# cordum-io/cordum

Measured on AMD Instinct MI355X. Metric: jobs dispatched/sec (whole node), higher is better.
Workload: dtype int64-bitset/int32 (control-plane integer path); 1 GPU; model=cordum control-plane dispatch pipeline (echo workers), global_batch=16384, seq_len=256, parallelism=shard1, rules=1024, workers_per_rank=1000, denied_jobs=14465

## Files before the change

cordum_amd/ops/hip/cordum_kernels.hip:

```cpp
#include <hip/hip_runtime.h>
#include <cstdint>

#define WAVE 64
#define BLOCK 256


template <int W, int JPT>
__global__ __launch_bounds__(BLOCK) void policy_first_match_kernel(
    const long long* __restrict__ rule_any,
    const long long* __restrict__ rule_all,
    const signed char* __restrict__ rule_secrets,
    const long long* __restrict__ rule_mcp,
    const unsigned char* __restrict__ rule_mcp_any,
    const long long* __restrict__ job_any,
    const long long* __restrict__ job_all,
    const unsigned char* __restrict__ job_secrets,
    const long long* __restrict__ job_mcp,
    const unsigned char* __restrict__ job_mcp_used,
    int* __restrict__ out_first,
    int R, int J, int rules_per_chunk)
{
    const int rule_chunk_begin = blockIdx.y * rules_per_chunk;
    const int rule_chunk_end = min(R, rule_chunk_begin + rules_per_chunk);
    constexpr int ANY_W = 7 * W;
// ... 1873 lines not shown
    #pragma unroll
    for (int t = 0; t < TJ; ++t) {
        const int job = (blockIdx.x * TJ + t) * 16 + (lane & 15);
        #pragma unroll
        for (int d = 0; d < 9; ++d) {
            unsigned long long w = 0;
            if (job < J)
                w = (unsigned long long)(d < 7 ? any_bits[(size_t)job * 7 + d]
                                               : all_bits[(size_t)job * 2 + (d - 7)]);
            const unsigned int slice = (unsigned int)(w >> shift) & 0xFFFFu;
            #pragma unroll
            for (int q = 0; q < 4; ++q)
                afrag[t][d][q] = (int)((((slice >> (4 * q)) & 0xFu) * 0x00204081u) & 0x01010101u);
        }
    }
    mfma_first_match_tiles<TJ>(afrag, b_pack, cards, rule_secrets, job_secrets,
                               tile_dims, out_first, J, R, tiles_per_chunk);
}

template <int TJ>
__global__ __launch_bounds__(BLOCK) void policy_first_match_mfma_cols_kernel(
    const long long* __restrict__ cols,
    int L, unsigned long long col_map,
    const signed char* __restrict__ b_pack,
    const int* __restrict__ cards,
    const signed char* __restrict__ rule_secrets,
    const unsigned char* __restrict__ job_secrets,
    const int* __restrict__ tile_dims,
    int* __restrict__ out_first,
    int J, int R, int tiles_per_chunk)
{
    const int lane = threadIdx.x % WAVE;
    const int shift = (lane >> 4) * 16;
    v4i afrag[TJ][9];
    #pragma unroll
    for (int t = 0; t < TJ; ++t) {
        const int job = (blockIdx.x * TJ + t) * 16 + (lane & 15);
        #pragma unroll
        for (int d = 0; d < 9; ++d) {
            const int c = (int)((col_map >> (4 * d)) & 0xFull);
            unsigned long long w = 0;
            if (c < L && job < J)
                w = (unsigned long long)cols[(size_t)job * L + c];
            const unsigned int slice = (unsigned int)(w >> shift) & 0xFFFFu;
            #pragma unroll
            for (int q = 0; q < 4; ++q)
                afrag[t][d][q] = (int)((((slice >> (4 * q)) & 0xFu) * 0x00204081u) & 0x01010101u);
        }
    }
    mfma_first_match_tiles<TJ>(afrag, b_pack, cards, rule_secrets, job_secrets,
                               tile_dims, out_first, J, R, tiles_per_chunk);
}


__global__ __launch_bounds__(BLOCK) void policy_gate_kernel(
    const int* __restrict__ first,
    const signed char* __restrict__ decisions,
    signed char* __restrict__ out_decision,
    int* __restrict__ denied_slots,
    int* __restrict__ denied_count,
    int* __restrict__ allowed_slots,
    int* __restrict__ allowed_count,
    int J, int R)
{
    const int j = blockIdx.x * BLOCK + threadIdx.x;
    const int lane = threadIdx.x % WAVE;
    gate_job(j, J, lane, first, decisions, R, out_decision,
             allowed_slots, allowed_count, denied_slots, denied_count);
}

__global__ __launch_bounds__(BLOCK) void policy_gate_full_kernel(
    const int* __restrict__ first,
    const signed char* __restrict__ decisions,
    signed char* __restrict__ out_decision,
    int* __restrict__ denied_slots,
    int* __restrict__ denied_count,
    int* __restrict__ allowed_slots,
    int* __restrict__ allowed_count,
    unsigned char* __restrict__ states,
    long long* __restrict__ deadlines,
    int* __restrict__ dlq_ring,
    int* __restrict__ dlq_head,
    int ring_size,
    int J, int R)
{
    const int j = blockIdx.x * BLOCK + threadIdx.x;
    const int lane = threadIdx.x % WAVE;
    const bool allowed = gate_job(j, J, lane, first, decisions, R, out_decision,
                                  allowed_slots, allowed_count, denied_slots, denied_count);
    deny_to_dlq(j < J && !allowed, j, lane, states, deadlines, dlq_ring, dlq_head, ring_size);
}

__global__ __launch_bounds__(BLOCK) void begin_tick_kernel(
    unsigned char* __restrict__ states, int B,
    int* __restrict__ counts, int ncounts,
    int* __restrict__ first)
{
    begin_slot(blockIdx.x * BLOCK + threadIdx.x, states, B, counts, ncounts, first);
}

__global__ void accumulate_counts_kernel(
    const int* __restrict__ counts, long long* __restrict__ acc, int n)
{
    const int t = threadIdx.x;
    if (t < n) acc[t] += (long long)counts[t];
}
// ... 856 lines not shown
    const int n = (int)counts.size(0);
    const int NW = (int)out_keys.size(0);
    TORCH_CHECK(w_active.size(0) == NW && w_maxp.size(0) == NW &&
                w_cpu.size(0) == NW && w_gpu.size(0) == NW, "worker table size mismatch");
    TORCH_CHECK(!first.has_value() || first->size(0) == B, "first must be [B]");
    const int blocks = (std::max(std::max(B, n), std::max(NW, 1)) + BLOCK - 1) / BLOCK;
    hipLaunchKernelGGL(tick_prologue_kernel, dim3(blocks), dim3(BLOCK), 0, cur_stream(),
        states.data_ptr<uint8_t>(), B, counts.data_ptr<int>(), n,
        first.has_value() ? first->data_ptr<int>() : (int*)nullptr,
        w_active.data_ptr<int>(), w_maxp.data_ptr<int>(),
        w_cpu.data_ptr<float>(), w_gpu.data_ptr<float>(),
        (unsigned long long*)out_keys.data_ptr<int64_t>(), NW);
}

void policy_first_match_mfma_bits_into(
    torch::Tensor any_bits, torch::Tensor all_bits,
    torch::Tensor b_pack, torch::Tensor cards,
    torch::Tensor rule_secrets, torch::Tensor job_secrets,
    torch::Tensor tile_dims, int64_t n_rules, torch::Tensor out, int64_t job_tiles)
{
    CHECK_DEV(any_bits); CHECK_DEV(b_pack);
    CHECK_CONTIG(any_bits); CHECK_CONTIG(all_bits);
    TORCH_CHECK(job_tiles == 1 || job_tiles == 2, "job_tiles must be 1 or 2");
    TORCH_CHECK(any_bits.dim() == 3 && any_bits.size(1) == 7 && any_bits.size(2) == 1 &&
                all_bits.dim() == 3 && all_bits.size(1) == 2 && all_bits.size(2) == 1,
                "MFMA K1 needs the 1-word vocab: any [J,7,1], all [J,2,1]");
    const int J = (int)any_bits.size(0), R = (int)n_rules;
    TORCH_CHECK(all_bits.size(0) == J && job_secrets.size(0) >= J && out.size(0) >= J,
                "job tensors must cover J");
    const int TJ = (int)job_tiles;
    const int Jt = ((J + 15) / 16 + TJ - 1) / TJ;
    const int Rt = (R + 15) / 16;
    if (J == 0 || R == 0) return;
    TORCH_CHECK(b_pack.size(0) >= Rt && tile_dims.size(0) >= Rt &&
                rule_secrets.size(0) >= Rt * 16 && cards.size(0) >= Rt * 16,
                "rule pack smaller than n_rules");
    int nchunks = std::max(1, std::min((Rt + 3) / 4, std::max(1, 2048 / std::max(Jt, 1))));
    const int tiles_per_chunk = (Rt + nchunks - 1) / nchunks;
    auto launch = [&](auto kernel) {
        hipLaunchKernelGGL(kernel, dim3(Jt, nchunks), dim3(BLOCK), 0, cur_stream(),
            (const long long*)any_bits.data_ptr<int64_t>(),
            (const long long*)all_bits.data_ptr<int64_t>(),
            (const signed char*)b_pack.data_ptr<int8_t>(),
            cards.data_ptr<int>(),
            (const signed char*)rule_secrets.data_ptr<int8_t>(),
            job_secrets.data_ptr<uint8_t>(),
            tile_dims.data_ptr<int>(),
            out.data_ptr<int>(), J, R, tiles_per_chunk);
    };
    if (TJ == 2) launch(policy_first_match_mfma_bits_kernel<2>);
    else launch(policy_first_match_mfma_bits_kernel<1>);
}

void policy_first_match_mfma_cols_into(
    torch::Tensor cols, int64_t col_map,
    torch::Tensor b_pack, torch::Tensor cards,
    torch::Tensor rule_secrets, torch::Tensor job_secrets,
    torch::Tensor tile_dims, int64_t n_rules, torch::Tensor out, int64_t job_tiles)
{
    CHECK_DEV(cols); CHECK_DEV(b_pack);
    CHECK_CONTIG(cols);
    TORCH_CHECK(job_tiles == 1 || job_tiles == 2, "job_tiles must be 1 or 2");
    TORCH_CHECK(cols.dim() == 2 && cols.scalar_type() == torch::kInt64 && cols.size(1) <= 9,
                "compact K1 needs cols [J,L] int64 with L <= 9 (1-word vocab)");
    const int J = (int)cols.size(0), R = (int)n_rules, L = (int)cols.size(1);
    TORCH_CHECK(job_secrets.size(0) >= J && out.size(0) >= J, "job tensors must cover J");
    TORCH_CHECK(col_map >= 0 && (col_map >> 36) == 0, "col_map holds 9 nibbles");
    unsigned map_dims = 0;
    int next_col = 0;
    for (int d = 0; d < 9; ++d) {
        const int c = (int)((col_map >> (4 * d)) & 0xF);
        if (c == 0xF) continue;
        TORCH_CHECK(c == next_col, "col_map must number the live dims 0..L-1 in ascending d");
        ++next_col;
        map_dims |= 1u << d;
    }
    TORCH_CHECK(next_col == L, "col_map names ", next_col, " columns, cols has ", L);
    const int TJ = (int)job_tiles;
    const int Jt = ((J + 15) / 16 + TJ - 1) / TJ;
    const int Rt = (R + 15) / 16;
    if (J == 0 || R == 0) return;
    TORCH_CHECK(b_pack.size(0) >= Rt && tile_dims.size(0) >= Rt &&
                rule_secrets.size(0) >= Rt * 16 && cards.size(0) >= Rt * 16,
                "rule pack smaller than n_rules");
    hipStreamCaptureStatus capturing = hipStreamCaptureStatusNone;
    TORCH_CHECK(hipStreamIsCapturing(cur_stream(), &capturing) == hipSuccess,
                "hipStreamIsCapturing failed");
    if (capturing == hipStreamCaptureStatusNone) {
        const torch::Tensor td = tile_dims.narrow(0, 0, Rt).cpu();
        const int* p = td.data_ptr<int>();
        unsigned scanned = 0;
        for (int rt = 0; rt < Rt; ++rt) scanned |= (unsigned)p[rt];
        TORCH_CHECK((scanned & 0x1FFu & ~map_dims) == 0,
                    "col_map lacks a dimension the packed policy scans (stale map?): "
                    "tile_dims union ", scanned & 0x1FFu, ", map dims ", map_dims);
    }
    int nchunks = std::max(1, std::min((Rt + 3) / 4, std::max(1, 2048 / std::max(Jt, 1))));
    const int tiles_per_chunk = (Rt + nchunks - 1) / nchunks;
    auto launch = [&](auto kernel) {
        hipLaunchKernelGGL(kernel, dim3(Jt, nchunks), dim3(BLOCK), 0, cur_stream(),
            (const long long*)cols.data_ptr<int64_t>(), L, (unsigned long long)col_map,
            (const signed char*)b_pack.data_ptr<int8_t>(),
            cards.data_ptr<int>(),
            (const signed char*)rule_secrets.data_ptr<int8_t>(),
            job_secrets.data_ptr<uint8_t>(),
            tile_dims.data_ptr<int>(),
            out.data_ptr<int>(), J, R, tiles_per_chunk);
    };
    if (TJ == 2) launch(policy_first_match_mfma_cols_kernel<2>);
    else launch(policy_first_match_mfma_cols_kernel<1>);
}

void gate_route(torch::Tensor first, torch::Tensor decisions, torch::Tensor out_decision,
                torch::Tensor denied_slots, torch::Tensor denied_count,
                torch::Tensor allowed_slots, torch::Tensor allowed_count,
                torch::Tensor states, torch::Tensor deadlines,
                torch::Tensor dlq_ring, torch::Tensor dlq_head,
                torch::Tensor pick, torch::Tensor order, torch::Tensor valid_count,
                torch::Tensor j_poolmask, torch::Tensor j_labels,
                int64_t full_mask, int64_t K,
                torch::Tensor routable_slots, torch::Tensor routable_widx,
                torch::Tensor routable_count, torch::Tensor extra_zero)
{
    CHECK_DEV(first);
    const int J = (int)first.size(0);
    TORCH_CHECK(out_decision.size(0) >= J && denied_slots.size(0) >= J &&
                allowed_slots.size(0) >= J && states.size(0) >= J &&
                deadlines.size(0) >= J && pick.size(0) >= J &&
                j_poolmask.size(0) >= J && j_labels.size(0) >= J &&
                routable_slots.size(0) >= J && routable_widx.size(0) >= J,
                "per-job tensors must cover J");
    TORCH_CHECK(K <= order.size(0), "K exceeds the order table");
    const int n_extra = (int)extra_zero.size(0);
    const int blocks = (std::max(std::max(J, n_extra), 1) + BLOCK - 1) / BLOCK;
    hipLaunchKernelGGL(gate_route_kernel, dim3(blocks), dim3(BLOCK), 0, cur_stream(),
        first.data_ptr<int>(), (const signed char*)decisions.data_ptr<int8_t>(),
        (signed char*)out_decision.data_ptr<int8_t>(),
        denied_slots.data_ptr<int>(), denied_count.data_ptr<int>(),
        allowed_slots.data_ptr<int>(), allowed_count.data_ptr<int>(),
        states.data_ptr<uint8_t>(), (long long*)deadlines.data_ptr<int64_t>(),
        dlq_ring.data_ptr<int>(), dlq_head.data_ptr<int>(), (int)dlq_ring.size(0),
        pick.data_ptr<int>(), order.data_ptr<int>(), valid_count.data_ptr<int>(),
        (const long long*)j_poolmask.data_ptr<int64_t>(),
        (const long long*)j_labels.data_ptr<int64_t>(),
        (long long)full_mask, (int)K,
        routable_slots.data_ptr<int>(), routable_widx.data_ptr<int>(),
        routable_count.data_ptr<int>(),
        extra_zero.data_ptr<int>(), n_extra,
        J, (int)decisions.size(0));
}

void tick_finish(torch::Tensor ctx_arena, torch::Tensor routable_slots,
                 torch::Tensor routable_widx, torch::Tensor routable_count,
                 torch::Tensor res_arena, torch::Tensor res_sum, int64_t stride,
                 torch::Tensor states, torch::Tensor attempts, torch::Tensor deadlines,
                 std::vector<int64_t> chain,
                 torch::Tensor w_active_local, int64_t nwl, int64_t my_rank,
                 torch::Tensor counts, torch::Tensor acc, int64_t capacity)
{
    CHECK_DEV(ctx_arena);
    TORCH_CHECK(capacity <= routable_slots.size(0) && capacity <= routable_widx.size(0),
                "capacity exceeds the routable lists");
    TORCH_CHECK(ctx_arena.numel() >= capacity * stride && res_arena.numel() >= capacity * stride &&
                res_sum.size(0) >= capacity && states.size(0) >= capacity,
// ... 852 lines not shown
          "gate + DENIED transition + DLQ ring append in one launch");
    m.def("begin_tick", &begin_tick, "tick prologue: PENDING re-admit + counter reset");
    m.def("accumulate_counts", &accumulate_counts, "fold tick counters into device accumulator");
    m.def("begin_tick_first", &begin_tick_first,
          "tick prologue that also primes the first-match buffer (INT_MAX)");
    m.def("least_loaded_pick_into", &least_loaded_pick_into,
          "K2 pick into a persistent buffer, skipping unconstrained jobs");
    m.def("policy_first_match_mfma_into", &policy_first_match_mfma_into,
          "K1 MFMA into a pre-primed buffer (no alloc/fill launches)");
    m.def("compact_routable_spread", &compact_routable_spread,
          "routable compaction with inline K2c spread");
    m.def("apply_transitions_chain_dyn", &apply_transitions_chain_dyn,
          "K5 chained targets in one launch (+ extra zero region)");
    m.def("compact_routable", &compact_routable, "routable-slot compaction");
    m.def("apply_transitions_dyn", &apply_transitions_dyn, "K5 with device-resident count");
    m.def("echo_execute_indexed_dyn", &echo_execute_indexed_dyn, "echo worker with device count");
    m.def("load_feedback", &load_feedback, "per-worker active-count histogram");
    m.def("run_readiness", &run_readiness, "K3 run/step readiness sweep");
    m.def("synthetic_fresh", &synthetic_fresh,
          py::call_guard<py::gil_scoped_release>(),
          "fused host synthetic-batch encoder");
    m.def("pack_jobs_mfma_dev", &pack_jobs_mfma_dev, "device job packing for the MFMA K1");
    m.def("synthetic_fresh_stamped", &synthetic_fresh_stamped,
          py::call_guard<py::gil_scoped_release>(),
          "host batch preparation in one call: synthetic dims + payload step stamp",
          py::arg("any_bits"), py::arg("all_bits"), py::arg("tenant_lut"),
          py::arg("topic_lut"), py::arg("risk_lut"), py::arg("req_lut"),
          py::arg("seed"), py::arg("step"), py::arg("dim_tenant"), py::arg("dim_topic"),
          py::arg("dim_risk"), py::arg("all_requires"), py::arg("payload"),
          py::arg("payload_words"), py::arg("threads") = 1, py::arg("isa_cap") = -1);
    m.def("synthetic_fresh_compact", &synthetic_fresh_compact,
          py::call_guard<py::gil_scoped_release>(),
          "synthetic_fresh_stamped into compact rows: one column per dim the policy reads",
          py::arg("cols"), py::arg("tenant_lut"), py::arg("topic_lut"),
          py::arg("risk_lut"), py::arg("req_lut"), py::arg("seed"), py::arg("step"),
          py::arg("col_of_tenant"), py::arg("col_of_topic"), py::arg("col_of_risk"),
          py::arg("col_of_requires"), py::arg("payload"), py::arg("payload_words"),
          py::arg("threads") = 1, py::arg("isa_cap") = -1);
    m.def("encoder_isa_level", [] { return cordum_enc::max_isa_level(); },
          "widest encoder ISA this CPU runs (0 baseline, 1 AVX2, 2 AVX-512DQ)");
    m.def("tick_prologue", &tick_prologue,
          "fused tick 1/5: PENDING re-admit + counter reset + first prime + worker keys");
    m.def("policy_first_match_mfma_bits_into", &policy_first_match_mfma_bits_into,
          "fused tick 3/5: K1 MFMA with A fragments built from the staged bit words",
          py::arg("any_bits"), py::arg("all_bits"), py::arg("b_pack"), py::arg("cards"),
          py::arg("rule_secrets"), py::arg("job_secrets"), py::arg("tile_dims"),
          py::arg("n_rules"), py::arg("out"), py::arg("job_tiles") = 1);
    m.def("policy_first_match_mfma_cols_into", &policy_first_match_mfma_cols_into,
          "fused tick 3/5, compact staging: K1 MFMA with A fragments built from the "
          "live-dimension columns",
          py::arg("cols"), py::arg("col_map"), py::arg("b_pack"), py::arg("cards"),
          py::arg("rule_secrets"), py::arg("job_secrets"), py::arg("tile_dims"),
          py::arg("n_rules"), py::arg("out"), py::arg("job_tiles") = 1);
    m.def("gate_route", &gate_route,
          "fused tick 4/5: gate + DENIED/DLQ + spread/exact pick + routable compaction");
    m.def("tick_finish", &tick_finish,
          "fused tick 5/5: echo + state chain + load feedback + counter fold");
    m.def("pack_by_dest", &pack_by_dest, "padded per-destination dispatch pack");
    m.def("pack_requeue", &pack_requeue, "redeliver last tick's requeue ring into the send segments");
    m.def("wf_sweep", &wf_sweep, "K3-WF readiness sweep + approval holds + condition/delay commits");
    m.def("wf_expand", &wf_expand, "K3-WF for_each/worker child expansion into the child arena");
    m.def("wf_apply", &wf_apply, "K3-WF child result application with failure injection");
    m.def("wf_apply_dead", &wf_apply_dead, "K3-WF dead-letter child application");
    m.def("wf_commit", &wf_commit, "K3-WF step aggregation + retry/backoff commit");
    m.def("wf_timeout_scan", &wf_timeout_scan, "K4-WF stale-step timeout scan");
    m.def("wf_readmit", &wf_readmit, "K3-WF continuous run re-admission from template");
    m.def("wf_status", &wf_status, "K3-WF run status roll-up");
    m.def("wf_grant", &wf_grant, "K3-WF host approval grants");
    m.def("wf_admit", &wf_admit, "K3-WF run admission into the lowest free slots");
    m.def("wf_cancel", &wf_cancel, "K3-WF generation-checked run cancellation");
    m.def("wf_retire", &wf_retire, "K3-WF completion records + quiescent slot release");
    m.def("wf_journal", &wf_journal, "K3-WF step-transition journal pass (observer)");
    m.def("wf_hold_scan", &wf_hold_scan, "K3-WF approval hold scan (open / expire / close holds)");
    m.def("wf_settle", &wf_settle, "K3-WF per-step-policy timeout + commit pass (replaces the scan/commit pair)");
    m.def("wf_cond_eval", &wf_cond_eval, "K3-WF predicate pass before the sweep (condition bits, guards -> SKIPPED)");
    m.def("wf_child_payload", &wf_child_payload, "K3-WF payload rows of the children emitted this tick");
    m.def("wf_apply_out", &wf_apply_out, "K3-WF child result application with step outputs");
    m.def("wf_hold_list", &wf_hold_list, "K3-WF ordered page of open approval holds");
    m.def("wf_decide", &wf_decide, "K3-WF generation-checked approval decisions");
    m.def("materialize_rq_payload", &materialize_rq_payload, "copy requeued payload rows into the rq arena");
    m.def("gather_payload_padded", &gather_payload_padded, "payload gather into padded send arena");
    m.def("echo_padded", &echo_padded, "region-valid echo over padded recv arena");
    m.def("apply_transitions_padded", &apply_transitions_padded, "K5 over padded slot list");
    m.def("load_feedback_padded", &load_feedback_padded, "padded per-worker load histogram");
    m.def("set_transition_lut", &set_transition_lut, "upload transition legality LUT");
    m.def("apply_transitions", &apply_transitions, "K5 batched state transitions");
    m.def("deadline_scan", &deadline_scan, "K4 deadline/staleness scan");
    m.def("echo_execute", &echo_execute, "device echo worker pool");
}
```

cordum_amd/ops/pipeline.py:

```python
from __future__ import annotations

import time
from dataclasses import dataclass
from typing import List, Optional

import torch
import torch.distributed as dist

from ..protocol.states import transition_lut
from ..safety import policy as pol
from . import get_ext
from .policy_compile import CompiledPolicy, JobBatch, JobEncoder, compile_policy, first_match_reference

UNSPECIFIED, PENDING, APPROVAL, SCHEDULED, DISPATCHED, RUNNING = 0, 1, 2, 3, 4, 5
SUCCEEDED, FAILED, CANCELLED, TIMEOUT, DENIED = 6, 7, 8, 9, 10

ALLOW_CODES = (1, 5)


@dataclass
class TickStats:
    completed: int = 0
    denied: int = 0
    unrouted: int = 0
# ... 423 lines not shown


def alloc_batch_staging(B: int, W: int, device=None, pin: bool = False):
    n64 = B * 7 * W + B * 2 * W + B * 4 * W
    nbytes = ((n64 * 8 + 2 * B + 7) // 8) * 8
    if pin:
        buf = torch.zeros(nbytes, dtype=torch.uint8).pin_memory()
    else:
        buf = torch.zeros(nbytes, dtype=torch.uint8, device=device)
    o = 0

    def take64(*shape):
        nonlocal o
        n = 1
        for s in shape:
            n *= s
        t = buf[o:o + n * 8].view(torch.int64).view(*shape)
        o += n * 8
        return t

    any_b = take64(B, 7, W)
    all_b = take64(B, 2, W)
    mcp_b = take64(B, 4, W)
    sec = buf[o:o + B]
    o += B
    used = buf[o:o + B]
    return JobBatch(any_b, all_b, sec, mcp_b, used), buf


def alloc_compact_staging(B: int, L: int, device=None, pin: bool = False):
    assert B >= 1 and 0 <= L <= 9
    nbytes = ((B * L * 8 + B + 7) // 8) * 8
    if pin:
        buf = torch.zeros(nbytes, dtype=torch.uint8).pin_memory()
    else:
        buf = torch.zeros(nbytes, dtype=torch.uint8, device=device)
    cols = buf[0:B * L * 8].view(torch.int64).view(B, L)
    sec = buf[B * L * 8:B * L * 8 + B]
    return cols, sec, buf


def alloc_result_block(B: int, device=None, pin: bool = False):
    nbytes = ((4 * B + 16 + B + 7) // 8) * 8
    if pin:
        buf = torch.zeros(nbytes, dtype=torch.uint8).pin_memory()
    else:
        buf = torch.zeros(nbytes, dtype=torch.uint8, device=device)
    sums = buf[0:4 * B].view(torch.int32)
    counts = buf[4 * B:4 * B + 16].view(torch.int32)
    dec = buf[4 * B + 16:5 * B + 16].view(torch.int8)
    return sums, counts, dec, buf


class DevicePipeline:
    def __init__(
        self,
        device: torch.device,
        batch_size: int = 16384,
        n_local_workers: int = 1000,
        n_rules: int = 1024,
        payload_words: int = 64,
        world_size: int = 1,
        rank: int = 0,
        n_batches: int = 8,
        policy: Optional[pol.SafetyPolicy] = None,
        seed: int = 7,
        backend: str = "ext",
        use_mfma: Optional[bool] = None,
        mfma_pack_on_device: bool = False,
        pad_cap: Optional[int] = None,
        unfused_tick: bool = False,
        k1_job_tiles: int = 2,
        compact_staging: Optional[bool] = None,
    ):
        self._k1_job_tiles = k1_job_tiles
        self._pad_cap_override = pad_cap
        self._unfused_tick = unfused_tick
        self._mfma_device_pack = mfma_pack_on_device
        device = torch.device(device)
        self.ext = _RefOps() if backend == "ref" else get_ext(required=True)
        self.device = device
        self.B = batch_size
        self.NWL = n_local_workers
        self.world = world_size
        self.rank = rank
        self.payload_words = payload_words

        self.ext.set_transition_lut(torch.tensor(transition_lut(), dtype=torch.uint8).flatten())

        policy = policy or make_synthetic_policy(n_rules, seed=seed)
        for w in (1, 2, 4):
            self.compiled = compile_policy(policy, words=w)
            if self.compiled.exact:
                break
        assert self.compiled.exact, "bench policy must compile exactly"
        self.cpol = self.compiled.to(device)

        self.batches: List[JobBatch] = []
        self.batch_bufs: List[torch.Tensor] = []
        self.payloads: List[torch.Tensor] = []
        for i in range(n_batches):
            jb = encode_synthetic_jobs(self.compiled, self.B, seed=seed * 1000 + i + rank * 77)
            dev_jb, dev_buf = alloc_batch_staging(self.B, self.compiled.words,
                                                  device=device)
            dev_jb.any_bits.copy_(jb.any_bits)
            dev_jb.all_bits.copy_(jb.all_bits)
            dev_jb.secrets.copy_(jb.secrets)
            dev_jb.mcp_bits.copy_(jb.mcp_bits)
            dev_jb.mcp_used.copy_(jb.mcp_used)
            self.batches.append(dev_jb)
            self.batch_bufs.append(dev_buf)
            g = torch.Generator().manual_seed(seed + i + rank * 131)
            payload = torch.randint(-(1 << 31), (1 << 31) - 1,
                                    (self.B * payload_words,), dtype=torch.int32, generator=g)
            self.payloads.append(payload.to(device))

        self.states = torch.zeros(self.B, dtype=torch.uint8, device=device)
        self.attempts = torch.zeros(self.B, dtype=torch.int32, device=device)
        self.deadlines = torch.full((self.B,), torch.iinfo(torch.int64).max,
                                    dtype=torch.int64, device=device)
        self.slots = torch.arange(self.B, dtype=torch.int32, device=device)

        NW = self.NWL
        g = torch.Generator().manual_seed(seed + 17 + rank)
        self.w_active_local = torch.zeros(NW, dtype=torch.int32, device=device)
        self.w_cpu_local = (torch.rand(NW, generator=g) * 50).to(device)
        self.w_gpu_local = (torch.rand(NW, generator=g) * 50).to(device)
        NWG = NW * self.world
        self.w_pool = (torch.arange(NWG, device=device, dtype=torch.int32) // NW)
        maxp_val = max(64, (4 * batch_size) // max(1, n_local_workers))
        self.w_maxp = torch.full((NWG,), maxp_val, dtype=torch.int32, device=device)
        self.w_labels = torch.zeros(NWG, dtype=torch.int64, device=device)
        self.w_active = torch.zeros(NWG, dtype=torch.int32, device=device)
        self.w_cpu = torch.zeros(NWG, dtype=torch.float32, device=device)
        self.w_gpu = torch.zeros(NWG, dtype=torch.float32, device=device)

        self.dlq_ring = torch.full((1 << 16,), -1, dtype=torch.int32, device=device)
        self.dlq_head = torch.zeros(1, dtype=torch.int32, device=device)

        NWG_ = self.NWL * self.world
        self.w_keys = torch.zeros(NWG_, dtype=torch.int64, device=device)
        self.order_buf = torch.arange(NWG_, dtype=torch.int32, device=device)
        self.valid_buf = torch.tensor([NWG_], dtype=torch.int32, device=device)

        self.j_poolmask = torch.full((self.B,), (1 << self.world) - 1,
                                     dtype=torch.int64, device=device)
        self.j_labels = torch.zeros(self.B, dtype=torch.int64, device=device)

        self.res_arena = torch.zeros(self.B * self.world * payload_words, dtype=torch.int32, device=device)
        (self.res_sums, self._counts, self.out_decision,
         self._res_block) = alloc_result_block(self.B, device=device)

        self.acc_counts = torch.zeros(4, dtype=torch.int64, device=device)
        self.first_buf = torch.full((self.B,), -1, dtype=torch.int32, device=device)
        self.pick_buf = torch.full((self.B,), -1, dtype=torch.int32, device=device)
        self.denied_slots = torch.zeros(self.B, dtype=torch.int32, device=device)
        self.denied_count = self._counts[0:1]
        self.allowed_count = self._counts[1:2]
        self.routable_count = self._counts[2:3]
        self.allowed_slots = torch.zeros(self.B, dtype=torch.int32, device=device)
        self.routable_slots = torch.zeros(self.B, dtype=torch.int32, device=device)
        self.routable_widx = torch.zeros(self.B, dtype=torch.int32, device=device)
        self._graph = None
        self._graphs = {}
        self._pad_graphs = None
        self._use_mfma = (
            backend != "ref"
            and device.type == "cuda"
            and world_size == 1
            and self.compiled.words == 1
            and self.compiled.n_rules <= 32768
            and int(self.compiled.mcp_any.sum()) == 0
        )
        if use_mfma is False:
            self._use_mfma = False
        if self._use_mfma and self._mfma_device_pack:
            from .policy_mfma import N_DIMS, pack_policy_mfma

            self.mfma_policy = pack_policy_mfma(self.compiled).to(device)
            self.mfma_a_packs = []
            if self._unfused_tick:
                Jt = (self.B + 15) // 16
                self.mfma_a_packs = [
                    torch.zeros(Jt, N_DIMS, 64, 16, dtype=torch.int8, device=device)
                    for _ in range(len(self.batches))
                ]
        elif self._use_mfma:
            from .policy_mfma import pack_jobs_mfma, pack_policy_mfma

            self.mfma_policy = pack_policy_mfma(self.compiled).to(device)
            self.mfma_a_packs = []
            for jb_host, jb_dev in zip(
                [encode_synthetic_jobs(self.compiled, self.B, seed=seed * 1000 + i + rank * 77)
                 for i in range(len(self.batches) if self._unfused_tick else 0)],
                self.batches
            ):
                a_pack, _ = pack_jobs_mfma(jb_host)
                self.mfma_a_packs.append(a_pack.to(device))
        self._fused_capable = device.type == "cuda" and self.world == 1 and backend != "ref"
        compact_ok = (self._fused_capable and self._use_mfma
                      and self._mfma_device_pack and not self._unfused_tick)
        if compact_staging and not compact_ok:
            raise ValueError("compact_staging needs the fused MFMA-from-bits tick "
                             "(single rank, 1-word vocabulary, CUDA, ext backend, "
                             "mfma_pack_on_device)")
        self._compact = compact_ok if compact_staging is None else bool(compact_staging)
        if self._compact:
            self._build_compact()
        self._tick = 0
        self.total_completed = 0
        self.total_denied = 0

    def _build_compact(self) -> None:
        from .policy_mfma import col_map, gather_live_cols, live_dims

        self._live = live_dims(self.mfma_policy)
        self._col_map = col_map(self._live)
        self.compact_cols: List[torch.Tensor] = []
        self.compact_secrets: List[torch.Tensor] = []
        self.compact_bufs: List[torch.Tensor] = []
        for jb in self.batches:
            cols, sec, buf = alloc_compact_staging(self.B, len(self._live),
                                                   device=self.device)
            cols.copy_(gather_live_cols(jb, self._live))
            sec.copy_(jb.secrets)
            self.compact_cols.append(cols)
            self.compact_secrets.append(sec)
            self.compact_bufs.append(buf)
        self._cgraphs = {}
        for name in ("_e2e_ccols", "_e2e_cbufs", "_e2e_ccolumns"):
            if hasattr(self, name):
                delattr(self, name)


    def _spread(self, pick):
        full_mask = (1 << self.world) - 1
        K = min(int(self.order_buf.shape[0]), 1024)
        self.ext.spread_pick(self.order_buf, self.valid_buf, self.j_poolmask,
                             self.j_labels, full_mask, pick, K)
        return pick

    def _refresh_order(self) -> None:
        if self._tick % 8 != 1:
            return
        self.order_buf.copy_(torch.argsort(self.w_keys).to(torch.int32))
        valid = ((self.w_keys >> 32) & 0xFFFFFFFF).ne(0xFFFFFFFE)
        self.valid_buf.copy_(valid.sum().to(torch.int32).reshape(1))

    def _fused_body(self, slot: int, compact: bool = False) -> None:
        assert not compact or self._compact, "compact staging is off"
        if self._unfused_tick:
            return self._unfused_body(slot)
        B = self.B
        ext = self.ext
        jb = self.batches[slot]
        full_mask = (1 << self.world) - 1
        ext.tick_prologue(self.states, self._counts,
                          self.first_buf if self._use_mfma else None,
                          self.w_active_local, self.w_maxp,
                          self.w_cpu_local, self.w_gpu_local, self.w_keys)
        ext.least_loaded_pick_into(self.w_pool, self.w_keys, self.w_labels,
                                   self.j_poolmask, self.j_labels,
                                   self.valid_buf, full_mask, self.pick_buf)
        if compact:
            ext.policy_first_match_mfma_cols_into(
                self.compact_cols[slot], self._col_map, self.mfma_policy.b_pack,
                self.mfma_policy.cards, self.mfma_policy.secrets,
                self.compact_secrets[slot], self.mfma_policy.tile_dims,
                self.compiled.n_rules, self.first_buf, self._k1_job_tiles)
            first = self.first_buf
        elif self._use_mfma:
            ext.policy_first_match_mfma_bits_into(
                jb.any_bits, jb.all_bits, self.mfma_policy.b_pack,
                self.mfma_policy.cards, self.mfma_policy.secrets, jb.secrets,
                self.mfma_policy.tile_dims, self.compiled.n_rules, self.first_buf,
                self._k1_job_tiles)
            first = self.first_buf
        else:
            first = ext.policy_first_match(
                self.cpol.any_masks, self.cpol.all_masks, self.cpol.secrets,
                self.cpol.mcp_masks, self.cpol.mcp_any,
                jb.any_bits, jb.all_bits, jb.secrets, jb.mcp_bits, jb.mcp_used, 0,
            )
        K = min(int(self.order_buf.shape[0]), 1024)
        ext.gate_route(first, self.cpol.decisions, self.out_decision,
                       self.denied_slots, self.denied_count,
                       self.allowed_slots, self.allowed_count,
                       self.states, self.deadlines, self.dlq_ring, self.dlq_head,
                       self.pick_buf, self.order_buf, self.valid_buf,
                       self.j_poolmask, self.j_labels, full_mask, K,
                       self.routable_slots, self.routable_widx,
                       self.routable_count, self.w_active_local)
        ext.tick_finish(self.payloads[slot], self.routable_slots,
                        self.routable_widx, self.routable_count,
                        self.res_arena[: B * self.payload_words], self.res_sums,
                        self.payload_words,
                        self.states, self.attempts, self.deadlines,
                        [SCHEDULED, DISPATCHED, RUNNING, SUCCEEDED],
                        self.w_active_local, self.NWL, self.rank,
                        self._counts, self.acc_counts, B)

    def _unfused_body(self, slot: int) -> None:
        B = self.B
        ext = self.ext
        jb = self.batches[slot]
        if self._use_mfma:
            ext.begin_tick_first(self.states, self._counts, self.first_buf)
            if self._mfma_device_pack:
                ext.pack_jobs_mfma_dev(jb.any_bits, jb.all_bits,
                                       self.mfma_a_packs[slot])
            ext.policy_first_match_mfma_into(
                self.mfma_a_packs[slot], self.mfma_policy.b_pack, self.mfma_policy.cards,
                self.mfma_policy.secrets, jb.secrets, self.mfma_policy.tile_dims,
                self.B, self.compiled.n_rules, self.first_buf,
            )
            first = self.first_buf
        else:
            ext.begin_tick(self.states, self._counts)
            first = ext.policy_first_match(
                self.cpol.any_masks, self.cpol.all_masks, self.cpol.secrets,
                self.cpol.mcp_masks, self.cpol.mcp_any,
                jb.any_bits, jb.all_bits, jb.secrets, jb.mcp_bits, jb.mcp_used, 0,
            )
        ext.policy_gate_full(first, self.cpol.decisions, self.out_decision,
                             self.denied_slots, self.denied_count,
                             self.allowed_slots, self.allowed_count,
                             self.states, self.deadlines,
                             self.dlq_ring, self.dlq_head)
        ext.worker_precompute_into(self.w_pool, self.w_active_local, self.w_maxp,
                                   self.w_cpu_local, self.w_gpu_local, self.w_keys)
        full_mask = (1 << self.world) - 1
        ext.least_loaded_pick_into(self.w_pool, self.w_keys, self.w_labels,
                                   self.j_poolmask, self.j_labels,
                                   self.valid_buf, full_mask, self.pick_buf)
        pick = self.pick_buf
        K = min(int(self.order_buf.shape[0]), 1024)
        ext.compact_routable_spread(self.allowed_slots, self.allowed_count, pick,
                                    self.order_buf, self.valid_buf,
                                    self.j_poolmask, self.j_labels, full_mask, K,
                                    self.routable_slots, self.routable_widx,
                                    self.routable_count)
        ext.echo_execute_indexed_dyn(self.payloads[slot], self.routable_slots,
                                     self.routable_count, self.res_arena[: B * self.payload_words],
                                     self.res_sums, self.payload_words, B)
        ext.apply_transitions_chain_dyn(self.states, self.attempts, self.deadlines,
                                        self.routable_slots, self.routable_count,
                                        [SCHEDULED, DISPATCHED, RUNNING, SUCCEEDED],
                                        self.w_active_local, B)
        ext.load_feedback(self.routable_widx, self.routable_count,
                          self.w_active_local, self.NWL, self.rank, B)
        ext.accumulate_counts(self._counts, self.acc_counts)

    def _ensure_graphs(self) -> None:
# ... 670 lines not shown
```

Before: 137.8 million jobs/s.

## Add rule-stationary MFMA first-match kernel with LDS best-rule tracking

```diff
diff --git a/cordum_amd/ops/hip/cordum_kernels.hip b/cordum_amd/ops/hip/cordum_kernels.hip
--- a/cordum_amd/ops/hip/cordum_kernels.hip
+++ b/cordum_amd/ops/hip/cordum_kernels.hip
@@ -1949,6 +1949,229 @@
                                tile_dims, out_first, J, R, tiles_per_chunk);
 }
 
+template <int L>
+struct K1WordsFromBits {
+    const long long* __restrict__ any_bits;
+    const long long* __restrict__ all_bits;
+    unsigned dim_mask;
+    __device__ __forceinline__ int dim_of(int slot) const {
+        int dim = 0, seen = 0;
+        #pragma unroll
+        for (int d = 0; d < 9; ++d)
+            if (dim_mask & (1u << d)) {
+                if (seen == slot) dim = d;
+                ++seen;
+            }
+        return dim;
+    }
+    __device__ __forceinline__ void load(int job, const int (&sdim)[L > 0 ? L : 1],
+                                         unsigned long long (&w)[L > 0 ? L : 1]) const {
+        #pragma unroll
+        for (int i = 0; i < L; ++i) {
+            const int d = sdim[i];
+            w[i] = (unsigned long long)(d < 7 ? any_bits[(size_t)job * 7 + d]
+                                              : all_bits[(size_t)job * 2 + (d - 7)]);
+        }
+    }
+};
+
+template <int L>
+struct K1WordsFromCols {
+    const long long* __restrict__ cols;
+    unsigned long long col_map;
+    __device__ __forceinline__ int dim_of(int slot) const {
+        int dim = 0;
+        #pragma unroll
+        for (int d = 0; d < 9; ++d)
+            if ((int)((col_map >> (4 * d)) & 0xFull) == slot) dim = d;
+        return dim;
+    }
+    __device__ __forceinline__ void load(int job, const int (&)[L > 0 ? L : 1],
+                                         unsigned long long (&w)[L > 0 ? L : 1]) const {
+        if (L > 0) __builtin_memcpy(&w[0], cols + (size_t)job * L, L * sizeof(long long));
+    }
+};
+
+template <int RW, int NS, class Words>
+__device__ __forceinline__ void mfma_first_match_rule_stationary(
+    const Words words,
+    const signed char* __restrict__ b_pack,
+    const int* __restrict__ cards,
+    const signed char* __restrict__ rule_secrets,
+    const unsigned char* __restrict__ job_secrets,
+    const int* __restrict__ tile_dims,
+    int* __restrict__ out_first,
+    int J, int R)
+{
+    static_assert(RW == 1 || RW == 2 || RW == 4, "a row's owned columns must fit one find-first-set");
+    constexpr int NA = NS > 0 ? NS : 1;
+    using rowbits_t = typename std::conditional<(RW > 2), unsigned long long, unsigned int>::type;
+    extern __shared__ int k1_rs_best[];
+    const int wave = __builtin_amdgcn_readfirstlane(threadIdx.x / WAVE);
+    const int lane = threadIdx.x % WAVE;
+    const int waves = blockDim.x / WAVE;
+    const int Rt = (R + 15) / 16;
+    const int Jt = (J + 15) / 16;
+    const int P = gridDim.x;
+    if ((int)blockIdx.x >= Jt) return;
+    const int T = (Jt - (int)blockIdx.x + P - 1) / P;
+    const int block_rule0 = blockIdx.y * waves * RW * 16;
+    const int rt0 = (blockIdx.y * waves + wave) * RW;
+    const bool later = blockIdx.y > 0;
+
+    for (int i = threadIdx.x; i < T * 16; i += blockDim.x) {
+        const int job = ((int)blockIdx.x + (i >> 4) * P) * 16 + (i & 15);
+        int v = INT_MIN;
+        if (job < J)
+            v = later ? __hip_atomic_load(&out_first[job], __ATOMIC_RELAXED, __HIP_MEMORY_SCOPE_AGENT)
+                      : INT_MAX;
+        k1_rs_best[i] = v;
+    }
+    __syncthreads();
+
+    const int col = lane & 15;
+    const int row_base = (lane >> 4) * 4;
+    const int shift = (lane >> 4) * 16;
+    const bool publisher = col < 4;
+    const int pub_row = row_base + (col & 3);
+
+    if (rt0 < Rt) {
+    int sdim[NA];
+    #pragma unroll
+    for (int i = 0; i < NS; ++i) sdim[i] = words.dim_of(i);
+
+    v4i bfrag[RW][NA];
+    int want[RW][NA];
+    int rsec[RW];
+    bool valid[RW];
+    #pragma unroll
+    for (int k = 0; k < RW; ++k) {
+        const bool live = rt0 + k < Rt;
+        const int rt = min(rt0 + k, Rt - 1);
+        const int rule = rt * 16 + col;
+        const unsigned dmask = live ? ((unsigned)tile_dims[rt] & 0x1FFu) : 0u;
+        valid[k] = live & (rule < R);
+        rsec[k] = (int)rule_secrets[rule];
+        #pragma unroll
+        for (int i = 0; i < NS; ++i) {
+            bfrag[k][i] = v4i{0, 0, 0, 0};
+            if (dmask & (1u << sdim[i]))
+                bfrag[k][i] = *(const v4i*)&b_pack[(((size_t)rt * 9 + sdim[i]) * 64 + lane) * 16];
+            want[k][i] = cards[rule * 9 + sdim[i]];
+        }
+    }
+    #pragma unroll
+    for (int k = 0; k < RW; ++k) {
+        #pragma unroll
+        for (int i = 0; i < NS; ++i)
+            if (sdim[i] < 7) want[k][i] = (want[k][i] == 0) ? -1 : 0;
+    }
+
+    unsigned long long w[NA];
+    unsigned char js[4];
+    auto load_tile = [&](int jt, unsigned long long (&tw)[NA], unsigned char (&tjs)[4]) {
+        words.load(min(jt * 16 + col, J - 1), sdim, tw);
+        #pragma unroll
+        for (int r = 0; r < 4; ++r)
+            tjs[r] = job_secrets[min(jt * 16 + row_base + r, J - 1)];
+    };
+
+    load_tile(blockIdx.x, w, js);
+    for (int n = 0; n < T; ++n) {
+        unsigned long long nw[NA];
+        unsigned char njs[4];
+        load_tile((int)blockIdx.x + min(n + 1, T - 1) * P, nw, njs);
+        int* const best = &k1_rs_best[n * 16 + pub_row];
+
+        if (!(later && __all(*best < rt0 * 16))) {
+            bool ok[RW][4];
+            #pragma unroll
+            for (int k = 0; k < RW; ++k) {
+                #pragma unroll
+                for (int r = 0; r < 4; ++r) ok[k][r] = true;
+            }
+            #pragma unroll
+            for (int i = 0; i < NS; ++i) {
+                const unsigned int slice = (unsigned int)(w[i] >> shift) & 0xFFFFu;
+                v4i afrag;
+                #pragma unroll
+                for (int q = 0; q < 4; ++q)
+                    afrag[q] = (int)((((slice >> (4 * q)) & 0xFu) * 0x00204081u) & 0x01010101u);
+                #pragma unroll
+                for (int k = 0; k < RW; ++k) {
+                    v4i zero = {0, 0, 0, 0};
+                    const v4i acc = __builtin_amdgcn_mfma_i32_16x16x64_i8(afrag, bfrag[k][i], zero, 0, 0, 0);
+                    #pragma unroll
+                    for (int r = 0; r < 4; ++r)
+                        ok[k][r] &= (acc[r] == want[k][i]) != (sdim[i] < 7);
+                }
+            }
+            rowbits_t mine = 0;
+            #pragma unroll
+            for (int r = 0; r < 4; ++r) {
+                rowbits_t bits = 0;
+                #pragma unroll
+                for (int k = 0; k < RW; ++k) {
+                    const bool pass = ok[k][r] & valid[k]
+                        & ((rsec[k] < 0) | (rsec[k] == (int)(signed char)js[r]));
+                    const unsigned long long m = __builtin_amdgcn_ballot_w64(pass);
+                    bits |= (rowbits_t)((unsigned int)(m >> shift) & 0xFFFFu) << (16 * k);
+                }
+                if ((col & 3) == r) mine = bits;
+            }
+            if (publisher && mine)
+                atomicMin(best, rt0 * 16 + (__ffsll((unsigned long long)mine) - 1));
+        }
+
+        #pragma unroll
+        for (int i = 0; i < NS; ++i) w[i] = nw[i];
+        #pragma unroll
+        for (int r = 0; r < 4; ++r) js[r] = njs[r];
+    }
+    }
+    __syncthreads();
+
+    for (int i = threadIdx.x; i < T * 16; i += blockDim.x) {
+        const int job = ((int)blockIdx.x + (i >> 4) * P) * 16 + (i & 15);
+        const int v = k1_rs_best[i];
+        if (job < J && v != INT_MAX && v >= block_rule0) atomicMin(&out_first[job], v);
+    }
+}
+
+template <int RW, int L, int WPB>
+__global__ __launch_bounds__(WPB * WAVE) void policy_first_match_mfma_bits_rs_kernel(
+    const long long* __restrict__ any_bits,
+    const long long* __restrict__ all_bits,
+    unsigned long long dim_mask,
+    const signed char* __restrict__ b_pack,
+    const int* __restrict__ cards,
+    const signed char* __restrict__ rule_secrets,
+    const unsigned char* __restrict__ job_secrets,
+    const int* __restrict__ tile_dims,
+    int* __restrict__ out_first,
+    int J, int R)
+{
+    mfma_first_match_rule_stationary<RW, L>(
+        K1WordsFromBits<L>{any_bits, all_bits, (unsigned)dim_mask},
+        b_pack, cards, rule_secrets, job_secrets, tile_dims, out_first, J, R);
+}
+
+template <int RW, int L, int WPB>
+__global__ __launch_bounds__(WPB * WAVE) void policy_first_match_mfma_cols_rs_kernel(
+    const long long* __restrict__ cols,
+    unsigned long long col_map,
+    const signed char* __restrict__ b_pack,
+    const int* __restrict__ cards,
+    const signed char* __restrict__ rule_secrets,
+    const unsigned char* __restrict__ job_secrets,
+    const int* __restrict__ tile_dims,
+    int* __restrict__ out_first,
+    int J, int R)
+{
+    mfma_first_match_rule_stationary<RW, L>(K1WordsFromCols<L>{cols, col_map},
+        b_pack, cards, rule_secrets, job_secrets, tile_dims, out_first, J, R);
+}
+
 
 __global__ __launch_bounds__(BLOCK) void policy_gate_kernel(
     const int* __restrict__ first,
@@ -2911,19 +3134,8 @@
     else launch(policy_first_match_mfma_bits_kernel<1>);
 }
 
-void policy_first_match_mfma_cols_into(
-    torch::Tensor cols, int64_t col_map,
-    torch::Tensor b_pack, torch::Tensor cards,
-    torch::Tensor rule_secrets, torch::Tensor job_secrets,
-    torch::Tensor tile_dims, int64_t n_rules, torch::Tensor out, int64_t job_tiles)
-{
-    CHECK_DEV(cols); CHECK_DEV(b_pack);
-    CHECK_CONTIG(cols);
-    TORCH_CHECK(job_tiles == 1 || job_tiles == 2, "job_tiles must be 1 or 2");
-    TORCH_CHECK(cols.dim() == 2 && cols.scalar_type() == torch::kInt64 && cols.size(1) <= 9,
-                "compact K1 needs cols [J,L] int64 with L <= 9 (1-word vocab)");
-    const int J = (int)cols.size(0), R = (int)n_rules, L = (int)cols.size(1);
-    TORCH_CHECK(job_secrets.size(0) >= J && out.size(0) >= J, "job tensors must cover J");
+static unsigned check_col_map(int64_t col_map, int L)
+{
     TORCH_CHECK(col_map >= 0 && (col_map >> 36) == 0, "col_map holds 9 nibbles");
     unsigned map_dims = 0;
     int next_col = 0;
@@ -2935,6 +3147,39 @@
         map_dims |= 1u << d;
     }
     TORCH_CHECK(next_col == L, "col_map names ", next_col, " columns, cols has ", L);
+    return map_dims;
+}
+
+static void check_map_covers_scan(const torch::Tensor& tile_dims, int Rt, unsigned map_dims,
+                                  const char* what)
+{
+    hipStreamCaptureStatus capturing = hipStreamCaptureStatusNone;
+    TORCH_CHECK(hipStreamIsCapturing(cur_stream(), &capturing) == hipSuccess,
+                "hipStreamIsCapturing failed");
+    if (capturing != hipStreamCaptureStatusNone) return;
+    const torch::Tensor td = tile_dims.narrow(0, 0, Rt).cpu();
+    const int* p = td.data_ptr<int>();
+    unsigned scanned = 0;
+    for (int rt = 0; rt < Rt; ++rt) scanned |= (unsigned)p[rt];
+    TORCH_CHECK((scanned & 0x1FFu & ~map_dims) == 0,
+                what, " lacks a dimension the packed policy scans (stale map?): "
+                "tile_dims union ", scanned & 0x1FFu, ", map dims ", map_dims);
+}
+
+void policy_first_match_mfma_cols_into(
+    torch::Tensor cols, int64_t col_map,
+    torch::Tensor b_pack, torch::Tensor cards,
+    torch::Tensor rule_secrets, torch::Tensor job_secrets,
+    torch::Tensor tile_dims, int64_t n_rules, torch::Tensor out, int64_t job_tiles)
+{
+    CHECK_DEV(cols); CHECK_DEV(b_pack);
+    CHECK_CONTIG(cols);
+    TORCH_CHECK(job_tiles == 1 || job_tiles == 2, "job_tiles must be 1 or 2");
+    TORCH_CHECK(cols.dim() == 2 && cols.scalar_type() == torch::kInt64 && cols.size(1) <= 9,
+                "compact K1 needs cols [J,L] int64 with L <= 9 (1-word vocab)");
+    const int J = (int)cols.size(0), R = (int)n_rules, L = (int)cols.size(1);
+    TORCH_CHECK(job_secrets.size(0) >= J && out.size(0) >= J, "job tensors must cover J");
+    const unsigned map_dims = check_col_map(col_map, L);
     const int TJ = (int)job_tiles;
     const int Jt = ((J + 15) / 16 + TJ - 1) / TJ;
     const int Rt = (R + 15) / 16;
@@ -2942,18 +3187,7 @@
     TORCH_CHECK(b_pack.size(0) >= Rt && tile_dims.size(0) >= Rt &&
                 rule_secrets.size(0) >= Rt * 16 && cards.size(0) >= Rt * 16,
                 "rule pack smaller than n_rules");
-    hipStreamCaptureStatus capturing = hipStreamCaptureStatusNone;
-    TORCH_CHECK(hipStreamIsCapturing(cur_stream(), &capturing) == hipSuccess,
-                "hipStreamIsCapturing failed");
-    if (capturing == hipStreamCaptureStatusNone) {
-        const torch::Tensor td = tile_dims.narrow(0, 0, Rt).cpu();
-        const int* p = td.data_ptr<int>();
-        unsigned scanned = 0;
-        for (int rt = 0; rt < Rt; ++rt) scanned |= (unsigned)p[rt];
-        TORCH_CHECK((scanned & 0x1FFu & ~map_dims) == 0,
-                    "col_map lacks a dimension the packed policy scans (stale map?): "
-                    "tile_dims union ", scanned & 0x1FFu, ", map dims ", map_dims);
-    }
+    check_map_covers_scan(tile_dims, Rt, map_dims, "col_map");
     int nchunks = std::max(1, std::min((Rt + 3) / 4, std::max(1, 2048 / std::max(Jt, 1))));
     const int tiles_per_chunk = (Rt + nchunks - 1) / nchunks;
     auto launch = [&](auto kernel) {
@@ -2969,6 +3203,132 @@
     if (TJ == 2) launch(policy_first_match_mfma_cols_kernel<2>);
     else launch(policy_first_match_mfma_cols_kernel<1>);
 }
+
+constexpr int K1_RS_BLOCKS = 256;
+constexpr int K1_RS_MIN_PARTS = 64;
+constexpr int K1_RS_MAX_TILES = 1024;
+
+struct K1RsLaunch { dim3 grid, block; size_t lds; };
+
+static K1RsLaunch k1_rs_launch(int J, int R, int RW, int WPB, int64_t job_parts)
+{
+    TORCH_CHECK(job_parts >= 0 && job_parts <= 4096, "job_parts must be 0 (auto) .. 4096");
+    const int Jt = (J + 15) / 16, Rt = (R + 15) / 16;
+    const int groups = (Rt + RW - 1) / RW;
+    const int waves = std::min(WPB, groups);
+    const int rows = (groups + waves - 1) / waves;
+    TORCH_CHECK(rows <= 65535, "too many rule tiles for one launch");
+    const int min_parts = (Jt + K1_RS_MAX_TILES - 1) / K1_RS_MAX_TILES;
+    const int P = job_parts > 0 ? (int)job_parts
+                                : std::max(min_parts, std::min(Jt, std::max(K1_RS_MIN_PARTS,
+                                                                            K1_RS_BLOCKS / rows)));
+    TORCH_CHECK(P >= min_parts, "job_parts leaves more than ", K1_RS_MAX_TILES, " job tiles per block");
+    const int T = (Jt + P - 1) / P;
+    return {dim3(P, rows), dim3(waves * WAVE), (size_t)T * 16 * sizeof(int)};
+}
+
+static int k1_rs_rule_tiles(int L, int64_t rule_tiles)
+{
+    TORCH_CHECK(rule_tiles == 0 || rule_tiles == 2 || (rule_tiles == 4 && L <= 4),
+                "rule_tiles must be 0 (auto), 2, or 4 with at most 4 dims");
+    return rule_tiles ? (int)rule_tiles : (L <= 4 ? 4 : 2);
+}
+
+#define K1_RS_CASE(KERNEL, RW_, L_) \
+    case L_: launch(KERNEL<RW_, L_, (RW_ == 4 ? 16 : 8)>); break
+#define K1_RS_DISPATCH(KERNEL, RW, L) \
+    if ((RW) == 4) { \
+        switch (L) { \
+        K1_RS_CASE(KERNEL, 4, 0); K1_RS_CASE(KERNEL, 4, 1); K1_RS_CASE(KERNEL, 4, 2); \
+        K1_RS_CASE(KERNEL, 4, 3); K1_RS_CASE(KERNEL, 4, 4); \
+        default: TORCH_CHECK(false, "no such K1 instantiation"); \
+        } \
+    } else { \
+        switch (L) { \
+        K1_RS_CASE(KERNEL, 2, 0); K1_RS_CASE(KERNEL, 2, 1); K1_RS_CASE(KERNEL, 2, 2); \
+        K1_RS_CASE(KERNEL, 2, 3); K1_RS_CASE(KERNEL, 2, 4); K1_RS_CASE(KERNEL, 2, 5); \
+        K1_RS_CASE(KERNEL, 2, 6); K1_RS_CASE(KERNEL, 2, 7); K1_RS_CASE(KERNEL, 2, 8); \
+        K1_RS_CASE(KERNEL, 2, 9); \
+        default: TORCH_CHECK(false, "no such K1 instantiation"); \
+        } \
+    }
+
+void policy_first_match_mfma_bits_rs_into(
+    torch::Tensor any_bits, torch::Tensor all_bits,
+    torch::Tensor b_pack, torch::Tensor cards,
+    torch::Tensor rule_secrets, torch::Tensor job_secrets,
+    torch::Tensor tile_dims, int64_t n_rules, torch::Tensor out, int64_t job_parts,
+    int64_t rule_tiles, int64_t dim_mask)
+{
+    CHECK_DEV(any_bits); CHECK_DEV(b_pack);
+    CHECK_CONTIG(any_bits); CHECK_CONTIG(all_bits);
+    TORCH_CHECK(any_bits.dim() == 3 && any_bits.size(1) == 7 && any_bits.size(2) == 1 &&
+                all_bits.dim() == 3 && all_bits.size(1) == 2 && all_bits.size(2) == 1,
+                "MFMA K1 needs the 1-word vocab: any [J,7,1], all [J,2,1]");
+    const int J = (int)any_bits.size(0), R = (int)n_rules;
+    TORCH_CHECK(all_bits.size(0) == J && job_secrets.size(0) >= J && out.size(0) >= J,
+                "job tensors must cover J");
+    TORCH_CHECK(dim_mask >= 0 && dim_mask <= 0x1FF, "dim_mask holds 9 bits");
+    const int L = __builtin_popcountll((unsigned long long)dim_mask);
+    const int Rt = (R + 15) / 16;
+    if (J == 0 || R == 0) return;
+    TORCH_CHECK(b_pack.size(0) >= Rt && tile_dims.size(0) >= Rt &&
+                rule_secrets.size(0) >= Rt * 16 && cards.size(0) >= Rt * 16,
+                "rule pack smaller than n_rules");
+    check_map_covers_scan(tile_dims, Rt, (unsigned)dim_mask, "dim_mask");
+    const int RW = k1_rs_rule_tiles(L, rule_tiles);
+    const K1RsLaunch ln = k1_rs_launch(J, R, RW, RW == 4 ? 16 : 8, job_parts);
+    auto launch = [&](auto kernel) {
+        hipLaunchKernelGGL(kernel, ln.grid, ln.block, ln.lds, cur_stream(),
+            (const long long*)any_bits.data_ptr<int64_t>(),
+            (const long long*)all_bits.data_ptr<int64_t>(),
+            (unsigned long long)dim_mask,
+            (const signed char*)b_pack.data_ptr<int8_t>(),
+            cards.data_ptr<int>(),
+            (const signed char*)rule_secrets.data_ptr<int8_t>(),
+            job_secrets.data_ptr<uint8_t>(),
+            tile_dims.data_ptr<int>(),
+            out.data_ptr<int>(), J, R);
+    };
+    K1_RS_DISPATCH(policy_first_match_mfma_bits_rs_kernel, RW, L)
+}
+
+void policy_first_match_mfma_cols_rs_into(
+    torch::Tensor cols, int64_t col_map,
+    torch::Tensor b_pack, torch::Tensor cards,
+    torch::Tensor rule_secrets, torch::Tensor job_secrets,
+    torch::Tensor tile_dims, int64_t n_rules, torch::Tensor out, int64_t job_parts,
+    int64_t rule_tiles)
+{
+    CHECK_DEV(cols); CHECK_DEV(b_pack);
+    CHECK_CONTIG(cols);
+    TORCH_CHECK(cols.dim() == 2 && cols.scalar_type() == torch::kInt64 && cols.size(1) <= 9,
+                "compact K1 needs cols [J,L] int64 with L <= 9 (1-word vocab)");
+    const int J = (int)cols.size(0), R = (int)n_rules, L = (int)cols.size(1);
+    TORCH_CHECK(job_secrets.size(0) >= J && out.size(0) >= J, "job tensors must cover J");
+    const unsigned map_dims = check_col_map(col_map, L);
+    const int Rt = (R + 15) / 16;
+    if (J == 0 || R == 0) return;
+    TORCH_CHECK(b_pack.size(0) >= Rt && tile_dims.size(0) >= Rt &&
+                rule_secrets.size(0) >= Rt * 16 && cards.size(0) >= Rt * 16,
+                "rule pack smaller than n_rules");
+    check_map_covers_scan(tile_dims, Rt, map_dims, "col_map");
+    const int RW = k1_rs_rule_tiles(L, rule_tiles);
+    const K1RsLaunch ln = k1_rs_launch(J, R, RW, RW == 4 ? 16 : 8, job_parts);
+    auto launch = [&](auto kernel) {
+        hipLaunchKernelGGL(kernel, ln.grid, ln.block, ln.lds, cur_stream(),
+            (const long long*)cols.data_ptr<int64_t>(), (unsigned long long)col_map,
+            (const signed char*)b_pack.data_ptr<int8_t>(),
+            cards.data_ptr<int>(),
+            (const signed char*)rule_secrets.data_ptr<int8_t>(),
+            job_secrets.data_ptr<uint8_t>(),
+            tile_dims.data_ptr<int>(),
+            out.data_ptr<int>(), J, R);
+    };
+    K1_RS_DISPATCH(policy_first_match_mfma_cols_rs_kernel, RW, L)
+}
+#undef K1_RS_DISPATCH
+#undef K1_RS_CASE
 
 void gate_route(torch::Tensor first, torch::Tensor decisions, torch::Tensor out_decision,
                 torch::Tensor denied_slots, torch::Tensor denied_count,
@@ -3927,6 +4287,19 @@
           py::arg("cols"), py::arg("col_map"), py::arg("b_pack"), py::arg("cards"),
           py::arg("rule_secrets"), py::arg("job_secrets"), py::arg("tile_dims"),
           py::arg("n_rules"), py::arg("out"), py::arg("job_tiles") = 1);
+    m.def("policy_first_match_mfma_bits_rs_into", &policy_first_match_mfma_bits_rs_into,
+          "fused tick 3/5: rule-stationary K1 MFMA from the staged bit words",
+          py::arg("any_bits"), py::arg("all_bits"), py::arg("b_pack"), py::arg("cards"),
+          py::arg("rule_secrets"), py::arg("job_secrets"), py::arg("tile_dims"),
+          py::arg("n_rules"), py::arg("out"), py::arg("job_parts") = 0,
+          py::arg("rule_tiles") = 0, py::arg("dim_mask") = 0x1FF);
+    m.def("policy_first_match_mfma_cols_rs_into", &policy_first_match_mfma_cols_rs_into,
+          "fused tick 3/5, compact staging: rule-stationary K1 MFMA from the "
+          "live-dimension columns",
+          py::arg("cols"), py::arg("col_map"), py::arg("b_pack"), py::arg("cards"),
+          py::arg("rule_secrets"), py::arg("job_secrets"), py::arg("tile_dims"),
+          py::arg("n_rules"), py::arg("out"), py::arg("job_parts") = 0,
+          py::arg("rule_tiles") = 0);
     m.def("gate_route", &gate_route,
           "fused tick 4/5: gate + DENIED/DLQ + spread/exact pick + routable compaction");
     m.def("tick_finish", &tick_finish,
diff --git a/cordum_amd/ops/pipeline.py b/cordum_amd/ops/pipeline.py
--- a/cordum_amd/ops/pipeline.py
+++ b/cordum_amd/ops/pipeline.py
@@ -499,6 +499,9 @@
     return sums, counts, dec, buf
 
 
+K1_RULE_STATIONARY_MAX_RULES = 16384
+
+
 class DevicePipeline:
     def __init__(
         self,
@@ -518,9 +521,11 @@
         pad_cap: Optional[int] = None,
         unfused_tick: bool = False,
         k1_job_tiles: int = 2,
+        k1_rule_stationary: Optional[bool] = None,
         compact_staging: Optional[bool] = None,
     ):
         self._k1_job_tiles = k1_job_tiles
+        self._k1_rule_stationary = k1_rule_stationary
         self._pad_cap_override = pad_cap
         self._unfused_tick = unfused_tick
         self._mfma_device_pack = mfma_pack_on_device
@@ -621,6 +626,9 @@
         )
         if use_mfma is False:
             self._use_mfma = False
+        if self._k1_rule_stationary is None:
+            self._k1_rule_stationary = (
+                self.compiled.n_rules <= K1_RULE_STATIONARY_MAX_RULES)
         if self._use_mfma and self._mfma_device_pack:
             from .policy_mfma import N_DIMS, pack_policy_mfma
 
@@ -644,6 +652,8 @@
             ):
                 a_pack, _ = pack_jobs_mfma(jb_host)
                 self.mfma_a_packs.append(a_pack.to(device))
+        if self._use_mfma:
+            self._k1_dim_mask()
         self._fused_capable = device.type == "cuda" and self.world == 1 and backend != "ref"
         compact_ok = (self._fused_capable and self._use_mfma
                       and self._mfma_device_pack and not self._unfused_tick)
@@ -709,19 +719,25 @@
         ext.least_loaded_pick_into(self.w_pool, self.w_keys, self.w_labels,
                                    self.j_poolmask, self.j_labels,
                                    self.valid_buf, full_mask, self.pick_buf)
+        rs = self._k1_rule_stationary
         if compact:
-            ext.policy_first_match_mfma_cols_into(
-                self.compact_cols[slot], self._col_map, self.mfma_policy.b_pack,
-                self.mfma_policy.cards, self.mfma_policy.secrets,
-                self.compact_secrets[slot], self.mfma_policy.tile_dims,
-                self.compiled.n_rules, self.first_buf, self._k1_job_tiles)
+            k1 = (ext.policy_first_match_mfma_cols_rs_into if rs
+                  else ext.policy_first_match_mfma_cols_into)
+            k1(self.compact_cols[slot], self._col_map, self.mfma_policy.b_pack,
+               self.mfma_policy.cards, self.mfma_policy.secrets,
+               self.compact_secrets[slot], self.mfma_policy.tile_dims,
+               self.compiled.n_rules, self.first_buf,
+               0 if rs else self._k1_job_tiles)
             first = self.first_buf
         elif self._use_mfma:
-            ext.policy_first_match_mfma_bits_into(
-                jb.any_bits, jb.all_bits, self.mfma_policy.b_pack,
-                self.mfma_policy.cards, self.mfma_policy.secrets, jb.secrets,
-                self.mfma_policy.tile_dims, self.compiled.n_rules, self.first_buf,
-                self._k1_job_tiles)
+            common = (jb.any_bits, jb.all_bits, self.mfma_policy.b_pack,
+                      self.mfma_policy.cards, self.mfma_policy.secrets, jb.secrets,
+                      self.mfma_policy.tile_dims, self.compiled.n_rules, self.first_buf)
+            if rs:
+                ext.policy_first_match_mfma_bits_rs_into(
+                    *common, dim_mask=self._k1_dim_mask())
+            else:
+                ext.policy_first_match_mfma_bits_into(*common, self._k1_job_tiles)
             first = self.first_buf
         else:
             first = ext.policy_first_match(
@@ -746,6 +762,15 @@
                         [SCHEDULED, DISPATCHED, RUNNING, SUCCEEDED],
                         self.w_active_local, self.NWL, self.rank,
                         self._counts, self.acc_counts, B)
+
+    def _k1_dim_mask(self) -> int:
+        cached = getattr(self, "_k1_dim_mask_of", None)
+        if cached is None or cached[0] is not self.mfma_policy:
+            from .policy_mfma import live_dims
+
+            mask = sum(1 << d for d in live_dims(self.mfma_policy))
+            self._k1_dim_mask_of = cached = (self.mfma_policy, mask)
+        return cached[1]
 
     def _unfused_body(self, slot: int) -> None:
         B = self.B
```

New measurement: 137.6 million jobs/s. About the same (-0.1%).
